# DankerMu/SHUD-up

Measured on AMD Instinct MI355X. Metric: element-flux-updates/sec (RHS evals × NumEle) at 1/2/4/8 GPUs; %HBM roofline, higher is better.
Workload: dtype f64

## Files before the change

shud-up_amd/csrc/shud_ele_packed.hip:

```cpp
#include <hip/hip_runtime.h>
#include <stdint.h>
#include <stdlib.h>

#include "shud_dev.h"
#include "shud_physics.h"

namespace shud {

typedef double v2d __attribute__((ext_vector_type(2)));
typedef int v4i __attribute__((ext_vector_type(4)));
template <class T>
__device__ __forceinline__ T ldnt(const T *p) { return __builtin_nontemporal_load(p); }
__device__ __forceinline__ double2 ldnt2(const double2 *p) {
    const v2d v = __builtin_nontemporal_load((const v2d *)p);
    return make_double2(v.x, v.y);
}
__device__ __forceinline__ int4 ldnt4(const int4 *p) {
    const v4i v = __builtin_nontemporal_load((const v4i *)p);
    return make_int4(v.x, v.y, v.z, v.w);
}
__device__ __forceinline__ void stnt2(double2 *p, double a, double b) {
    v2d v;
    v.x = a;
    v.y = b;
    __builtin_nontemporal_store(v, (v2d *)p);
}
template <class T>
__device__ __forceinline__ const T *at(const T *b, uint32_t off) { return (const T *)((const char *)b + off); }
template <class T>
__device__ __forceinline__ T *atw(T *b, uint32_t off) { return (T *)((char *)b + off); }

__device__ __forceinline__ bool nan_or_inf(double x) { return __builtin_isfpclass(x, 0x0003 | 0x0004 | 0x0200); }
__device__ __forceinline__ bool bad_nonneg(double x) {
    return __builtin_isfpclass(x, 0x0003 | 0x0004 | 0x0008 | 0x0010 | 0x0200);
}

__device__ __forceinline__ const double *riv_y_at(const YView &Y, int r) {
    return r < Y.n_own_riv ? Y.y + 3 * (size_t)Y.n_own + r : Y.griv + (r - Y.n_own_riv);
}

__device__ __forceinline__ int cf_ibc(int cf) { return (int)(int8_t)(cf & 0xff); }
__device__ __forceinline__ int cf_iss(int cf) { return (cf >> 8) & 3; }
__device__ __forceinline__ int cf_nseg(int cf) { return (cf >> 10) & 63; }
__device__ __forceinline__ int cf_class(int cf) { return (int)(((unsigned)cf >> 16) & 0x7fffu); }

template <int MODE>
__device__ __forceinline__ double ugw_pk(const DevMesh &m, double ygw_raw, int ibc, int j) {
    if (ibc == 0) return MODE == 0 ? ygw_raw : rmax(0.0, ygw_raw);
    if (ibc > 0) return m.eybc[ibc];
    return m.ugw_stale[j];
}

constexpr int LDS_CLS_MAX = kLdsClassMax;
constexpr int CF_LDS_STRIDE = CF_STRIDE;

constexpr int kEleWaves = 5;
constexpr int kEleWavesSh = 7;
constexpr bool kShareOn(bool lct, bool gh, bool lake, int hyb, bool diag) {
    return lct && !gh && !lake && hyb == 0 && !diag;
}
constexpr int kEleWavesOf(bool lct, int lspk, bool gh, bool lake, int hyb, bool diag, bool fu1, bool open) {
    return (kShareOn(lct, gh, lake, hyb, diag) && lspk) ? (fu1 ? kEleWavesSh : 6)
           : (kShareOn(lct, gh, lake, hyb, diag) && !open) ? 6 : kEleWaves;
}
constexpr int kEleBS = 256;
static_assert(kEleBS == kShareTile, "edge sharing pairs elements within one workgroup's tile");
static_assert(2 * kEleBS * 8 + kEleBS <= kPowTabDoubles * 8, "edge-sharing slots fit the pow tables' LDS region");
struct OwnRec {
    int4 mt;
    double2 zz, snp, stl, fu, csv;
    double ysf, yus, ygw;
    int sfl;
};
template <bool FU1, bool GH>
__device__ __forceinline__ OwnRec load_own(const DevPacked &p, const YView &Y, int i, int cur) {
    const int nown = Y.n_own;
    const uint32_t o16 = (uint32_t)i << 4, o8 = (uint32_t)i << 3;
    OwnRec o;
    o.mt = *at(p.meta, o16);
    o.zz = *at(p.zz, o16);
    o.ysf = GH ? Y.sf(i) : *at(Y.y, o8);
    o.yus = GH ? Y.us(i) : *at(Y.y + nown, o8);
    o.ygw = GH ? Y.gw(i) : *at(Y.y + 2 * (size_t)nown, o8);
    o.snp = ldnt2(at(p.s_np, o16));
    o.stl = ldnt2(at(p.s_tl, o16));
    if (FU1) { o.fu.x = 1.0; o.fu.y = 1.0; } else o.fu = ldnt2(at(p.s_fu, o16));
    o.csv = ldnt2(at(p.cs[cur], o16));
    o.sfl = *at(p.seg_first, (uint32_t)i << 2);
    return o;
}

constexpr int kTabBatch = 8;
template <int BS>
__device__ __forceinline__ void tab_issue(const DevPacked &p, double (&tv)[kTabBatch]) {
    const int nt2 = (p.ntab + 1) >> 1;
#pragma unroll
    for (int k = 0; k < kTabBatch / 2; k++) {
        const int t = (int)threadIdx.x + k * BS;
        const double2 v = t < nt2 ? ((const double2 *)p.ctab)[t] : make_double2(0., 0.);
        tv[2 * k] = v.x;
        tv[2 * k + 1] = v.y;
    }
}
template <int BS>
__device__ __forceinline__ void tab_store(const DevPacked &p, const double (&tv)[kTabBatch], double *lct) {
    const int nt2 = (p.ntab + 1) >> 1;
#pragma unroll
    for (int k = 0; k < kTabBatch / 2; k++) {
        const int t = (int)threadIdx.x + k * BS;
        if (t < nt2) ((double2 *)lct)[t] = make_double2(tv[2 * k], tv[2 * k + 1]);
    }
    for (int t = (int)threadIdx.x + kTabBatch / 2 * BS; t < nt2; t += BS)
        ((double2 *)lct)[t] = ((const double2 *)p.ctab)[t];
}
__device__ __forceinline__ int tile_of(int per8, int b) { return (b & 7) * per8 + (b >> 3); }
__device__ __forceinline__ int tile_of(int per8) { return tile_of(per8, (int)blockIdx.x); }
__device__ __forceinline__ bool share_idle_wave(bool act) {
    if (__builtin_amdgcn_ballot_w64(act)) return false;
    __syncthreads();
    __syncthreads();
    return true;
}

struct HaloWait;
template <int MODE, bool HALO>
__device__ __forceinline__ void qd_pre(const DevMesh &m, const DevPacked &p, const YView &Y, int r, int n_int,
                                       const HaloWait *hw);
__device__ __forceinline__ int qd_split(int b, int nb_q, int q0, int *e) {
    if (nb_q && b >= q0 && b < q0 + nb_q) return b - q0;
    *e = b < q0 ? b : b - nb_q;
    return -1;
}

template <int MODE, bool OPEN, bool DIAG, bool FU1, bool LCT, bool LAKE, bool GH, int HYB = 0, int LSP = 0, int BS = 256>
__device__ __forceinline__ void ele_body(const DevMesh &m, const DevPacked &p, const YView &Y, double *__restrict__ dy,
                                         int i, int cur, const DevDiag &dg, const DevLake &lk, const double *lct,
                                         const OwnRec &own);

template <int MODE, bool OPEN, bool DIAG, bool FU1, bool LCT, bool LAKE, bool GH, int HYB = 0, int LSPK = 0>
__global__ void __launch_bounds__(kEleBS, kEleWavesOf(LCT, LSPK, GH, LAKE, HYB, DIAG, FU1, OPEN))
shud_ele_kernel_packed(DevMesh m, DevPacked p, YView Y, double *__restrict__ dy, int i0, int n_compute, int cur,
                       DevDiag dg, DevLake lk, int per8, int nb_q, int q0) {
    extern __shared__ double lct[];
    int eb = (int)blockIdx.x;
    const int qb = qd_split((int)blockIdx.x, nb_q, q0, &eb);
    if (qb >= 0) {
        const int r = qb * kEleBS + (int)threadIdx.x;
        if (r < p.nqd) qd_pre<MODE, false>(m, p, Y, r, 0, nullptr);
        return;
    }
    const int i = i0 + tile_of(per8, eb) * kEleBS + (int)threadIdx.x;
    const bool act = i < n_compute;
    double tv[kTabBatch];
    if (LCT) tab_issue<kEleBS>(p, tv);
    OwnRec own;
    if (act) own = load_own<FU1, GH>(p, Y, i, cur);
    if (LCT) {
        tab_store<kEleBS>(p, tv, lct);
        __syncthreads();
    }
    if (kShareOn(LCT, GH, LAKE, HYB, DIAG) && LSPK != 0 && share_idle_wave(act)) return;
    if (act) ele_body<MODE, OPEN, DIAG, FU1, LCT, LAKE, GH, HYB, LCT ? LSPK : 0>(m, p, Y, dy, i, cur, dg, lk, lct, own);
}

template <int MODE, bool OPEN, bool DIAG, bool FU1, bool GH>
__global__ void __launch_bounds__(1024, 4)
shud_ele_kernel_packed_big(DevMesh m, DevPacked p, YView Y, double *__restrict__ dy, int i0, int n_compute, int cur,
                           DevDiag dg, DevLake lk, int per8) {
    extern __shared__ double lct[];
    const int i = i0 + tile_of(per8) * 1024 + (int)threadIdx.x;
    const bool act = i < n_compute;
    double tv[kTabBatch];
    tab_issue<1024>(p, tv);
    OwnRec own;
    if (act) own = load_own<FU1, GH>(p, Y, i, cur);
    tab_store<1024>(p, tv, lct);
    __syncthreads();
    if (act) ele_body<MODE, OPEN, DIAG, FU1, true, false, GH, 0, 0, 1024>(m, p, Y, dy, i, cur, dg, lk, lct, own);
}

__device__ __forceinline__ void halo_wait(const DevMesh &m, const HaloWait &hw, int i) {
    if (hw.epoch == 0) return;
    bool late = false;
    if (__lane_id() == 0) {
        const unsigned long long t0 = wall_clock64();
        while (__hip_atomic_load(hw.flag, __ATOMIC_RELAXED, __HIP_MEMORY_SCOPE_AGENT) < hw.epoch) {
            __builtin_amdgcn_s_sleep(8);
            if (wall_clock64() - t0 > hw.timeout) { late = true; break; }
        }
    }
    __builtin_amdgcn_fence(__ATOMIC_ACQUIRE, "agent");
    asm volatile("s_waitcnt vmcnt(0)" ::: "memory");
    report_w(m.err, late, 0x80u, 7, i);
}
template <int MODE, bool OPEN, bool FU1, int LSPK = 0>
__global__ void __launch_bounds__(256, (LSPK && FU1 && !OPEN) ? kEleWavesSh : kEleWaves)
shud_ele_kernel_packed_fold(DevMesh m, DevPacked p, YView Y, double *__restrict__ dy, int n_int, int n_all, int cur,
                            DevDiag dg, int per8, int nb_int, HaloWait hw, int nb_q, int q0) {
    extern __shared__ double lct[];
    const DevLake lk{};
    int b = (int)blockIdx.x;
    const int qb = qd_split((int)blockIdx.x, nb_q, q0, &b);
    if (qb >= 0) {
        const int r = qb * 256 + (int)threadIdx.x;
        qd_pre<MODE, true>(m, p, Y, r < p.nqd ? r : -1, n_int, &hw);
        return;
    }
    if (b < nb_int) {
        const int i = tile_of(per8, b) * 256 + (int)threadIdx.x;
        const bool act = i < n_int;
        double tv[kTabBatch];
        tab_issue<256>(p, tv);
        OwnRec own;
        if (act) own = load_own<FU1, false>(p, Y, i, cur);
        tab_store<256>(p, tv, lct);
        __syncthreads();
        if (LSPK != 0 && share_idle_wave(act)) return;
        if (act) ele_body<MODE, OPEN, false, FU1, true, false, false, 0, LSPK>(m, p, Y, dy, i, cur, dg, lk, lct, own);
        return;
    }
    const int i = n_int + (b - nb_int) * 256 + (int)threadIdx.x;
    const bool act = i < n_all;
    double tv[kTabBatch];
    tab_issue<256>(p, tv);
    halo_wait(m, hw, act ? i : n_int);
    OwnRec own;
    if (act) own = load_own<FU1, true>(p, Y, i, cur);
    tab_store<256>(p, tv, lct);
    __syncthreads();
    if (act) ele_body<MODE, OPEN, false, FU1, true, false, true, 0, LSPK ? 2 : 0>(m, p, Y, dy, i, cur, dg, lk, lct, own);
}
__global__ void shud_halo_flag_kernel(unsigned long long *flag, unsigned long long epoch) {
    if (threadIdx.x == 0) {
        __builtin_amdgcn_fence(__ATOMIC_RELEASE, "agent");
        asm volatile("s_waitcnt vmcnt(0)" ::: "memory");
        __hip_atomic_store(flag, epoch, __ATOMIC_RELAXED, __HIP_MEMORY_SCOPE_AGENT);
    }
}
__global__ void shud_spin_kernel(unsigned long long ticks) {
    if (threadIdx.x == 0) {
        const unsigned long long t0 = wall_clock64();
        while (wall_clock64() - t0 < ticks) __builtin_amdgcn_s_sleep(4);
    }
}
__global__ void shud_copy_f64_kernel(double *__restrict__ dst, const double *__restrict__ src, size_t n) {
    for (size_t k = blockIdx.x * (size_t)blockDim.x + threadIdx.x; k < n; k += (size_t)gridDim.x * blockDim.x)
        dst[k] = src[k];
}

__device__ __forceinline__ double hsel(const double (&v)[4], int k) {
    return k == 1 ? v[0] : k == 2 ? v[1] : k == 3 ? v[2] : v[3];
}
__device__ __forceinline__ void hload(const DevPacked &p, int i, double (&v)[4]) {
    v[1] = 0.; v[2] = 0.; v[3] = 0.;
    if (p.hs == 1) {
        v[0] = p.hv[i];
        return;
    }
    const double2 a = *(const double2 *)(p.hv + (size_t)p.hs * i);
    v[0] = a.x; v[1] = a.y;
    if (p.hs == 4) {
        const double2 b = *(const double2 *)(p.hv + (size_t)p.hs * i + 2);
        v[2] = b.x; v[3] = b.y;
    }
}

template <int MODE, bool OPEN, bool DIAG, bool FU1, bool LCT, bool LAKE, bool GH, int HYB, int LSP, int BS>
__device__ __forceinline__ void ele_body(const DevMesh &m, const DevPacked &p, const YView &Y, double *__restrict__ dy,
                                         int i, int cur, const DevDiag &dg, const DevLake &lk, const double *lct,
                                         const OwnRec &own) {
    const int NEl = m.num_ele;
    const int nown = Y.n_own;
    const uint32_t o16 = (uint32_t)i << 4, o8 = (uint32_t)i << 3;
    (void)o16;
    const int4 mt = own.mt;
    const double2 zz = own.zz;
    const double ysf_raw = own.ysf, yus_raw = own.yus, ygw_raw = own.ygw;
    const int cf = mt.w;
    const int cid = cf_class(cf), ibc = cf_ibc(cf);
    const bool is_lake = LAKE && cf < 0;
    const double2 snp = own.snp, stl = own.stl;
    const double etp = stl.y;
    const double2 fu = own.fu;
    const double2 csv = own.csv;
#define REPORT(c, bit, slot, cnt) report_w(m.err, (c), (bit), (slot), i, (cnt))
#define REPORT_ET(c, bit) (rep |= (c) ? (uint32_t)(bit) : 0u)
#define CL(f) (LCT ? lct[cid * CF_LDS_STRIDE + CfPos<CF_##f>::v] : p.ctab[cid * CF_STRIDE + CfPos<CF_##f>::v])
#define CDIV(a, F) cdiv(a, CL(F), CL(r_##F))
    double hvo[4] = {0., 0., 0., 0.};
    if (HYB == 1) hvo[0] = p.hv[i];
    else if (HYB == 2) hload(p, i, hvo);
#define CLH(f) ((HYB && p.hslot1[CF_##f]) ? (HYB == 1 ? hvo[0] : hsel(hvo, p.hslot1[CF_##f])) : CL(f))
#define CDIV_SY(a) ((HYB && p.hslot1[CF_Sy]) ? (a) / (HYB == 1 ? hvo[0] : hsel(hvo, p.hslot1[CF_Sy])) : CDIV(a, Sy))

    double usf = ysf_raw, uus = yus_raw;
    if (MODE == 1) { usf = (usf >= 0.) ? usf : 0.; uus = (uus >= 0.) ? uus : 0.; }
    const double ugw = ugw_pk<MODE>(m, ygw_raw, ibc, i);
    const double zs = zz.x, zb = zz.y;
    const double aq = zs - zb;

    double ekh, deficit, theta, satn, satkr;
    if (is_lake) {
        ekh = CLH(KsatH); deficit = 0.; satn = 1.; theta = CL(ThetaS); satkr = 1.0;
    } else {
        ekh = eff_kh(ugw, aq, CLH(macD), CLH(macKsatH), CLH(vAreaF), CLH(KsatH));
        REPORT(ekh < 0. || ekh > 1e9, 0x02u, 1, false);
        deficit = aq - ugw;
        const double ThS = CL(ThetaS), ThR = CL(ThetaR);
        if (deficit <= 0.) { deficit = 0.; satn = 1.; theta = ThS; }
        else { theta = uus / deficit * ThS; satn = CDIV(theta - ThR, dTh); }
        if (satn > 0.99) { satn = 1.0; satkr = 1.0; theta = ThS; }
        else if (satn <= K_ZERO) { satn = 0.; satkr = 0.; theta = ThR; }
        else {
            const double *pt = (LCT ? lct : p.ctab) + p.pt_off;
            satkr = sat_kfun(satn, CL(ex1), CL(ex2), pt, pt + kPowTabLogDoubles);
        }
    }

    const int sfl = own.sfl;
    const int sfirst = sfl & ((LSP || DIAG || !LCT) ? 0x03ffffff : 0x7fffffff);
    const bool lai_on = sfl < 0;
    const int iss = cf_iss(cf), nseg = cf_nseg(cf);
    const double infD = CL(infD), ThR = CL(ThetaR);
    const double infK = CL(infKsatV);
    const double fu_surf = fu.x, fu_sub = fu.y;

    double Es = 0., Eu = 0., Eg = 0., Tu = 0., Tg = 0., eic = csv.y, ibeta = 0.;
    if (is_lake) {
        eic = 0.;
        if (DIAG) { dg.q_es[i] = 0.; dg.q_eu[i] = 0.; dg.q_eg[i] = 0.; dg.q_tu[i] = 0.; dg.q_tg[i] = 0.;
                    dg.q_eta[i] = 0. + snp.y + 0.; }
    } else if (MODE == 0) {
        const double satn_prev = csv.x;
        const double va = CL(VegFrac), vb = 1. - va, pj = CL(pj);
        const double pet = snp.y, ptr = stl.x;
        ibeta = soil_moisture_stress(CDIV(satn_prev * CL(dTh) - ThR, fcmr));
        Es = rmin(rmax(0., usf), pet) * vb;
        if (Es < pet) {
            if (ugw > aq - infD) { Eg = rmin(rmax(0., ugw), pet - Es) * pj * vb; Eu = 0.; }
            else { Eg = 0.; Eu = rmin(rmax(0., uus), ibeta * (pet - Es)) * pj * vb; }
        }
        if (lai_on) {
            if (eic >= ptr) { Tg = Tu = 0.; eic = ptr * pj * va; }
            else if (ugw > aq - CLH(RzD)) { Tg = rmin(rmax(0., ugw), (ptr - eic)) * pj * va; Tu = 0.; }
            else { Tg = 0.; Tu = rmin(rmax(0., uus), ibeta * (ptr - eic)) * pj * va; }
        } else { Tg = Tu = eic = 0.; }
        const double trans = Tg + Tu, evapo = Eu + Eg + Es, eta = eic + evapo + trans;
        uint32_t rep = 0;
        REPORT_ET(eta > etp * 2., 0x10u);
        const bool neg = bad_nonneg(Es) || bad_nonneg(Eu) || bad_nonneg(Eg) || bad_nonneg(Tu) || bad_nonneg(Tg);
        REPORT_ET(neg, 0x04u);
        REPORT_ET(!neg && (nan_or_inf(eta) || nan_or_inf(evapo) || nan_or_inf(trans)), 0x08u);
        if (__builtin_amdgcn_ballot_w64(rep != 0)) {
            report_w(m.err, rep & 0x04u, 0x04u, 2, i);
            report_w(m.err, rep & 0x08u, 0x08u, 3, i);
            report_w(m.err, rep & 0x10u, 0x10u, 4, i, true);
        }
        if (DIAG) { dg.q_es[i] = Es; dg.q_eu[i] = Eu; dg.q_eg[i] = Eg; dg.q_tu[i] = Tu; dg.q_tg[i] = Tg;
                    dg.q_eta[i] = eta; dg.i_beta[i] = ibeta; }
    }
    stnt2(atw(p.cs[cur ^ 1], o16), satn, eic);

    double qi = 0., qex = 0., qr = 0.;
    if (!is_lake) {
        const double kmax = CL(kmax);
        const double av = usf + snp.x;
        if (ugw + uus > aq || deficit < uus) {
            qex = fabs(ugw + uus - aq) / aq * kmax;
        } else if (av > 0. && deficit > infD) {
            const double grad = 1. + CDIV(av, infD);
            double ek;
            if (av > kmax) ek = CL(ekA) + CL(ekB) * satn;
            else if (av > infK) ek = satkr * infK * CL(omh) + CL(ekB) * satn;
            else ek = satkr * infK * CL(omh);
            qi = rmin(av, rmax(0., grad * ek));
        }
        const double KV = CLH(KsatV);
        if (!(ugw > aq - infD && uus < deficit)) {
            double grad = 0.;
            if (theta > ThR && !(uus <= K_EPSILON)) {
                grad = CDIV(theta - ThR, fcmr);
                grad = rmax(grad, 0.);
            }
            if (!(infK <= 0. || KV <= 0.)) {
                const double ku = infK * satkr;
                qr = grad * ((ku * KV) * (deficit + ugw) / (deficit * KV + ugw * ku));
            }
        }
    }
    const double q_infil = qi * fu_surf, q_exfil = qex * fu_surf;
    const double q_rech = is_lake ? 0. : qr * fu_sub;

    const double dsf_head = snp.x - q_infil + q_exfil;
    const double dgw_head = q_rech - q_exfil;
    typedef __attribute__((address_space(3))) volatile double lds_vd;
    lds_vd *lsp = LSP ? (lds_vd *)(lct + p.ntab) + threadIdx.x : nullptr;
    typedef __attribute__((address_space(3))) volatile int lds_vi;
    lds_vi *lspi = LSP ? (lds_vi *)(lct + p.ntab + kLspN * kEleBS) + threadIdx.x : nullptr;
    if (LSP) {
        lsp[0] = Es; lsp[kEleBS] = Eg; lsp[2 * kEleBS] = Tg; lsp[3 * kEleBS] = dsf_head; lsp[4 * kEleBS] = dgw_head;
        lspi[0] = cf;
    }
    if (i < nown) __builtin_nontemporal_store(is_lake ? 0. : CDIV_SY(q_infil - q_rech - Eu - Tu), atw(dy + nown, o8));

    const double dep = CLH(depression), rgh = CLH(rough);
    double qe2r_surf = 0., qe2r_sub = 0.;
    if (nseg) {
        const double isf_seg = rmax(0., usf - q_infil + q_exfil);
        for (int k = sfirst, k1 = k + nseg; k < k1; k++) {
            const uint32_t k16 = (uint32_t)k << 4;
            const double2 lc = *at(p.sg_lc, k16);
            const int rr = *at(p.sg_r, (uint32_t)k << 2);
            const double2 dk = p.rrec[2 * (size_t)rr], rx = p.rrec[2 * (size_t)rr + 1];
            const int rbc = __builtin_bit_cast(int2, rx.y).x;
            const double bt = rx.x;
            double yr = GH ? Y.riv(rr) : *at(Y.y + 3 * (size_t)nown, (uint32_t)rr << 3);
            if (MODE == 1) yr = (yr >= 0.) ? yr : 0.;
            if (rbc > 0) yr = m.rybc[rbc];
            const double rdep = dk.x, L = lc.x;
            const double qs = weir_jtoi(zs, isf_seg, zs - rdep, yr, zs + 0.0, lc.y, L, dep);
            const double qg = r2e_gw(yr, zs - rdep, ugw, zb, ekh, dk.y, L, bt) * fu_sub;
            *atw(p.qseg2, k16) = make_double2(qs, qg);
            qe2r_surf += -qs;
            qe2r_sub += -qg;
        }
    }
    if (DIAG) {
        dg.q_infil[i] = q_infil; dg.q_exfil[i] = q_exfil; dg.q_recharge[i] = q_rech;
        dg.e_ic[i] = eic; dg.u_satn[i] = satn; dg.eff_kh[i] = ekh;
        dg.qe2r_surf[i] = qe2r_surf; dg.qe2r_sub[i] = qe2r_sub;
    }
    if (i >= nown) return;

    bool nan_q = false;
    const double isf = usf < 0. ? 0. : usf;
    const double area = ldnt(at(p.area, o8));
    const int n_edges = is_lake ? 0 : 3;
    constexpr bool SH = kShareOn(LCT, GH, LAKE, HYB, DIAG) && LSP != 0 && BS == kEleBS;
    constexpr bool DEC = !SH && LCT && !LAKE && HYB == 0 && BS == kEleBS && (LSP == 1 || DIAG);
    [[maybe_unused]] const uint32_t evo = (uint32_t)sfl >> kEvoShift;
    auto edge = [&](int s, int j, double &qsf, double &q, uint32_t &sh) __attribute__((always_inline)) {
        const int nb = s == 0 ? mt.x : s == 1 ? mt.y : mt.z;
        const int nc = nb >= 0 ? nb : i;
        const uint32_t n16 = (uint32_t)nc << 4, n8 = (uint32_t)nc << 3;
        const double2 g = ldnt2(at(p.ged, o16 + (uint32_t)s * ((uint32_t)NEl << 4)));
        const double2 nzz = *at(p.zz, n16);
        const int ncf = *at((const int *)p.meta + 3, n16);
        const double nsf_raw = GH ? Y.sf(nc) : *at(Y.y, n8);
        const double ngw_raw = GH ? Y.gw(nc) : *at(Y.y + 2 * (size_t)nown, n8);
        const double B = g.x, d2n = g.y;
        const Recip R2 = recip_nr(d2n);
        qsf = 0.; q = 0.; sh = 0u;
        const double dep_e = SH ? (double)((lds_vd *)lct)[cid * CF_LDS_STRIDE + CfPos<CF_depression>::v] : dep;
        const double rgh_e = SH ? (double)((lds_vd *)lct)[cid * CF_LDS_STRIDE + CfPos<CF_rough>::v] : rgh;
        const int cn = cf_class(ncf);
#define CN(f) (LCT ? lct[cn * CF_LDS_STRIDE + CfPos<CF_##f>::v] : p.ctab[cn * CF_STRIDE + CfPos<CF_##f>::v])
        double hvn[4] = {0., 0., 0., 0.};
        if (HYB == 1 && p.hnb) hvn[0] = p.hv[nc];
        else if (HYB == 2 && p.hnb) hload(p, nc, hvn);
#define CNH(f) ((HYB && p.hslot1[CF_##f]) ? (HYB == 1 ? hvn[0] : hsel(hvn, p.hslot1[CF_##f])) : CN(f))
        if (LAKE && nb >= 0 && ncf < 0) {
            const int l = lk.lake_of[nb];
            const double zl = lk.bathy_y[lk.bathy_off[l]];
            const double yl = Y.y[lk.y_off + l];
            const double nsf = yl < 0. ? 0. : yl;
            qsf = weir_jtoi(zl, nsf, zs, isf, zs, 0.6, B, 0.01);
            const double dhg = (ugw + zb) - (yl + zl);
            if (dhg > 0. && ugw <= 0.02) q = 0.;
            else if (dhg < 0. && yl <= 0.02) q = 0.;
            else {
                const double ymg = (rmax(ugw, 0.) + rmax(yl, 0.)) * .5;
                const double grad = div_nr(dhg, R2);
                const double kmean = 0.5 * (ekh + CNH(KsatH));
                q = kmean * grad * ymg * B;
            }
            lk.bank_qs[(size_t)j * NEl + i] = qsf;
            lk.bank_qg[(size_t)j * NEl + i] = q;
        } else if (nb >= 0) {
            double nsf = nsf_raw;
            if (MODE == 1) nsf = (nsf >= 0.) ? nsf : 0.;
            nsf = nsf < 0. ? 0. : nsf;
            const double zsn = nzz.x;
            const double dh = (isf + zs) - (nsf + zsn);
            [[maybe_unused]] const bool dh_nz = dh != 0., dh_ok = dh == dh;
            double ym = ((isf + zs) > (nsf + zsn)) ? ((isf > dep_e) ? isf : 0.) : ((nsf > dep_e) ? nsf : 0.);
            ym = rmin(ym, K_MAXYSURF);
            bool mu = false;
            if (ym > 0.) {
                const double s = div_nr(dh, R2);
                if (s > 0 && isf <= 0) qsf = 0.;
                else if (s < 0 && nsf <= 0) qsf = 0.;
                else { qsf = manning(ym * B, 0.5 * (rgh_e + CNH(rough)), ym, s); mu = true; }
            }
            const double ugn = ugw_pk<MODE>(m, ngw_raw, cf_ibc(ncf), nb);
            const double zbn = nzz.y;
            const double dhg = (ugw + zb) - (ugn + zbn);
            [[maybe_unused]] const bool dhg_nz = dhg != 0., dhg_ok = dhg == dhg;
            bool zq = true;
            if (dhg > 0. && ugw <= 0.02) q = 0.;
            else if (dhg < 0. && ugn <= 0.02) q = 0.;
            else {
                const double ekn = eff_kh(ugn, zsn - zbn, CNH(macD), CNH(macKsatH), CNH(vAreaF), CNH(KsatH));
                const double ymg = (rmax(ugw, 0.) + rmax(ugn, 0.)) * .5;
                const double grad = div_nr(dhg, R2);
                const double kmean = 0.5 * (ekh + ekn);
                q = kmean * grad * ymg * B;
                zq = false;
            }
            if constexpr (SH) sh = (mu && dh_nz ? 1u : 0u) | (!zq && dhg_nz ? 2u : 0u) | (dh_ok && dhg_ok ? 4u : 0u);
        } else if (OPEN) {
            const double d2e = m.dist2edge[(SH ? evo_ref(evo, s) : j) * NEl + i];
            if (isf > dep_e) {
                const double s = isf / d2e * 0.5;
                if (s > 0.) qsf = sqrt(s) * cbrt(isf * isf * isf * isf * isf) * B / rgh_e;
            }
            if (ugw > dep_e * 10.) {
                const double grad = ugw / d2e * 0.5;
                if (grad > 0.) q = ekh * grad;
            }
        }
#undef CN
#undef CNH
    };
    double sumsurf = qe2r_surf, sumsub = qe2r_sub;
    auto add = [&](int j, double qsf, double q) __attribute__((always_inline)) {
        const double qsb = q * fu_sub;
        if (MODE == 0) nan_q |= nan_or_inf(qsf) || nan_or_inf(qsb);
        sumsurf += qsf;
        sumsub += qsb;
        if (DIAG) { dg.qele_surf[j * NEl + i] = qsf; dg.qele_sub[j * NEl + i] = qsb; }
    };
    if constexpr (!SH) {
#pragma unroll 1
        for (int j = 0; j < n_edges; j++) {
            double qsf, q;
            uint32_t sh;
            edge(DEC ? evo_stored(evo, j) : j, j, qsf, q, sh);
            add(j, qsf, q);
        }
    } else {
        typedef __attribute__((address_space(3))) volatile unsigned char lds_vb;
        lds_vd *xq = (lds_vd *)(lct + p.pt_off);
        lds_vb *xf = (lds_vb *)(lct + p.pt_off + 2 * kEleBS);
        const int tid = (int)threadIdx.x;
        __syncthreads();
        {
            double qsf, q;
            uint32_t sh;
            edge(0, 0, qsf, q, sh);
            xq[tid] = qsf;
            xq[kEleBS + tid] = q;
            xf[tid] = (unsigned char)sh;
        }
        __syncthreads();
        double a1, b1, a2 = 0., b2 = 0.;
        {
            uint32_t sh;
            edge(1, 1, a1, b1, sh);
        }
        bool own2 = true;
        if (evo & (kEvoRcv2 >> kEvoShift)) {
            const int rt = mt.z - (i - tid);
            if (rt >= 0 && rt < kEleBS) {
                const uint32_t f = xf[rt];
                if (f & 4u) {
                    const double a = xq[rt], b = xq[kEleBS + rt];
                    a2 = (f & 1u) ? -a : a;
                    b2 = (f & 2u) ? -b : b;
                    own2 = false;
                }
            }
        }
        if (__builtin_amdgcn_ballot_w64(own2)) {
            if (own2) {
                uint32_t sh;
                edge(2, 2, a2, b2, sh);
            }
        }
        const double a0 = xq[tid], b0 = xq[kEleBS + tid];
        const uint32_t s0 = evo & 3u;
        const bool sw = (evo & 4u) != 0;
        const double la = s0 == 0 ? a1 : a0, lb = s0 == 0 ? b1 : b0;
        const double ha = s0 == 2 ? a1 : a2, hb = s0 == 2 ? b1 : b2;
        add(0, s0 == 0 ? a0 : s0 == 1 ? a1 : a2, s0 == 0 ? b0 : s0 == 1 ? b1 : b2);
        add(1, sw ? ha : la, sw ? hb : lb);
        add(2, sw ? la : ha, sw ? lb : hb);
    }
    if (DIAG && is_lake)
        for (int j = 0; j < 3; j++) { dg.qele_surf[j * NEl + i] = 0.; dg.qele_sub[j * NEl + i] = 0.; }
    if (MODE == 0) REPORT(nan_q, 0x01u, 0, false);

    double dsf, dgw;
    const Recip RA = recip_nr(area);
    if (LSP) {
        const double es = lsp[0], eg = lsp[kEleBS], tg = lsp[2 * kEleBS], dsh = lsp[3 * kEleBS], dgh = lsp[4 * kEleBS];
        dsf = dsh - div_nr(sumsurf, RA) - es;
        dgw = dgh - div_nr(sumsub, RA) - eg - tg;
    } else {
        dsf = dsf_head - div_nr(sumsurf, RA) - Es;
        dgw = dgw_head - div_nr(sumsub, RA) - Eg - Tg;
    }
    const int cf_t = LSP ? lspi[0] : cf;
    const int ibc_t = LSP ? cf_ibc(cf_t) : ibc, iss_t = LSP ? cf_iss(cf_t) : iss;
    if (ibc_t > 0) dgw = 0;
    else if (ibc_t < 0) dgw += div_nr(m.eqbc[-ibc_t], RA);
    if (iss_t == 1) dsf += zero_over(area);
    else if (iss_t == 2) dgw += zero_over(area);
    dgw = CDIV_SY(dgw);
    if (LSP ? (LAKE && cf_t < 0) : is_lake) { dsf = 0.; dgw = 0.; }
#undef CL
#undef CLH
#undef CDIV_SY
    __builtin_nontemporal_store(dsf, atw(dy, o8));
    __builtin_nontemporal_store(dgw, atw(dy + 2 * (size_t)nown, o8));
    if (DIAG) { dg.qele_surf_tot[i] = sumsurf; dg.qele_sub_tot[i] = sumsub; }
#undef REPORT
#undef REPORT_ET
}

struct RivP {
    double w0, bs, len, slope, d2d, n, depth;
    int down, bc;
};
__device__ __forceinline__ int2 rv_ib(double x) { return __builtin_bit_cast(int2, x); }
__device__ __forceinline__ RivP riv_load(const DevPacked &p, int r) {
    const double2 *q = p.rv + 4 * (size_t)r;
    const double2 a = q[0], b = q[1], c = q[2], d = q[3];
    const int2 ib = rv_ib(d.y);
    RivP o;
    o.w0 = a.x; o.bs = a.y; o.len = b.x; o.slope = b.y; o.d2d = c.x; o.n = c.y; o.depth = d.x;
    o.down = ib.x; o.bc = ib.y;
    return o;
}
__device__ __forceinline__ RivGeom riv_geom_p(const RivP &q, double y) { return riv_geom(q.w0, q.bs, q.len, y); }
template <int MODE>
__device__ __forceinline__ double riv_stage_p(const DevMesh &m, const YView &Y, int r, int bc, double *yg) {
    double yr = Y.riv(r);
    if (MODE == 1) yr = (yr >= 0.) ? yr : 0.;
    *yg = yr;
    return bc > 0 ? m.rybc[bc] : yr;
}
__device__ __forceinline__ double riv_down_p(const RivP &q, double uq, const RivGeom &g, double ud, double ddepth,
                                             double dslope) {
    if (q.down >= 0) {
        const double smean = (q.slope + dslope) * 0.5;
        const double s = ((uq - q.depth) - (ud - ddepth)) / q.d2d + smean;
        const double R = (g.csperem <= K_ZERO) ? 0. : (g.csarea / g.csperem);
        return manning(g.csarea, q.n, R, s);
    } else if (q.down >= -3) {
        const double s = q.slope + uq * 2. / q.len;
        const double R = (g.csperem <= 0.) ? 0. : (g.csarea / g.csperem);
        return manning(g.csarea, q.n, R, s);
    }
    return g.csarea * sqrt(K_GRAV * uq) * 60.;
}
__device__ __forceinline__ double riv_down_outlet(const RivP &q, double uq, const RivGeom &g) {
    return riv_down_p(q, uq, g, 0., 0., 0.);
}
template <int MODE, bool HALO>
__device__ __forceinline__ void qd_pre(const DevMesh &m, const DevPacked &p, const YView &Y, int r, int n_int,
                                       const HaloWait *hw) {
    const int rr = r < 0 ? 0 : r;
    const RivP q = riv_load(p, rr);
    const int d = q.down >= 0 ? q.down : rr;
    if (HALO) {
        const bool ghost = r >= 0 && (r >= Y.n_own_riv || d >= Y.n_own_riv);
        if (__builtin_amdgcn_ballot_w64(ghost)) halo_wait(m, *hw, n_int);
    }
    if (r < 0) return;
    double yg;
    const double ur = riv_stage_p<MODE>(m, Y, r, q.bc, &yg);
    const RivGeom g = riv_geom_p(q, yg);
    const double2 bd = p.rv[4 * (size_t)d + 1], dd = p.rv[4 * (size_t)d + 3];
    double ydg;
    const double ud = riv_stage_p<MODE>(m, Y, d, rv_ib(dd.y).y, &ydg);
    p.qdown[r] = riv_down_p(q, ur, g, ud, dd.x, bd.y);
}

struct __attribute__((packed, aligned(4))) Int4u { int x, y, z, w; };
struct __attribute__((packed, aligned(4))) Int2u { int x, y; };

template <int MODE, bool DIAG, int SB, bool QD>
__device__ __forceinline__ void riv_body(const DevMesh &m, const DevPacked &p, const YView &Y, double *__restrict__ dy,
                                         const DevDiag &dg, int r) {
    const RivP q = riv_load(p, r);
    const int4 ru = p.rv_u[r];
    const int seg0 = ru.x, nseg = ru.y & 0xffff, upc = ru.y >> 16;
    double yg;
    const double ur = riv_stage_p<MODE>(m, Y, r, q.bc, &yg);
    const RivGeom g = riv_geom_p(q, yg);
    double qdown = 0.;
    if (QD) {
        qdown = p.qdown[r];
    } else {
        const int d = q.down >= 0 ? q.down : r;
        const double2 bd = p.rv[4 * (size_t)d + 1], dd = p.rv[4 * (size_t)d + 3];
        const int bcd = rv_ib(dd.y).y;
        double ydg;
        const double ud = riv_stage_p<MODE>(m, Y, d, bcd, &ydg);
        qdown = riv_down_p(q, ur, g, ud, dd.x, bd.y);
    }
    auto up_term = [&](int u) {
        if (QD) return -p.qdown[u];
        const RivP qu = riv_load(p, u);
        double yu;
        const double uu = riv_stage_p<MODE>(m, Y, u, qu.bc, &yu);
        return -riv_down_p(qu, uu, riv_geom_p(qu, yu), ur, q.depth, q.slope);
    };
    double qup = 0.;
    if (upc < 3) {
        if (upc > 0) qup += up_term(ru.z);
        if (upc > 1) qup += up_term(ru.w);
    } else {
        for (int k0 = ru.z, k1 = ru.z + ru.w; k0 < k1; k0 += 8) {
            int uv[8];
#pragma unroll
            for (int j = 0; j < 8; j++) uv[j] = m.up_idx[k0 + j < k1 ? k0 + j : k0];
#pragma unroll
            for (int j = 0; j < 8; j++)
                if (k0 + j < k1) qup += up_term(uv[j]);
        }
    }
    double qsurf = 0., qsub = 0.;
    for (int k0 = seg0, k1 = seg0 + nseg; k0 < k1; k0 += SB) {
        int raw[SB], ps[SB];
#pragma unroll
        for (int c = 0; c + 4 <= SB; c += 4) {
            const Int4u v = *reinterpret_cast<const Int4u *>(m.rseg_pos + k0 + c);
            raw[c] = v.x; raw[c + 1] = v.y; raw[c + 2] = v.z; raw[c + 3] = v.w;
        }
        if constexpr (SB % 4 == 2) {
            const Int2u v = *reinterpret_cast<const Int2u *>(m.rseg_pos + k0 + SB - 2);
            raw[SB - 2] = v.x; raw[SB - 1] = v.y;
        }
#pragma unroll
        for (int j = 0; j < SB; j++) ps[j] = k0 + j < k1 ? raw[j] : raw[0];
        double2 qv[SB];
#pragma unroll
        for (int j = 0; j < SB; j++) qv[j] = p.qseg2[ps[j]];
#pragma unroll
        for (int j = 0; j < SB; j++)
            if (k0 + j < k1) { qsurf += qv[j].x; qsub += qv[j].y; }
    }
    const double qbc = (q.bc < 0) ? m.rqbc[-q.bc] : 0.0;
    double dv;
    if (q.bc > 0) dv = 0.;
    else if (MODE == 0) {
        dv = (-qup - qsurf - qsub - qdown + qbc) / q.len;
        if (dv < -1. * g.csarea) dv = -1. * g.csarea;
        dv = da_to_dy(dv, g.topw, q.bs);
    } else {
        dv = (-qup - qsurf - qsub - qdown + qbc) / g.toparea;
    }
    dy[3 * Y.n_own + r] = dv;
    if (DIAG) { dg.qriv_down[r] = qdown; dg.qriv_up[r] = qup; dg.qriv_surf[r] = qsurf; dg.qriv_sub[r] = qsub; }
}
template <int MODE, bool DIAG, int SB, bool QD>
__global__ void __launch_bounds__(256)
shud_riv_kernel_packed(DevMesh m, DevPacked p, YView Y, double *__restrict__ dy, DevDiag dg, int per8) {
    const int r = tile_of(per8) * 256 + (int)threadIdx.x;
    if (r >= Y.n_own_riv) return;
    riv_body<MODE, DIAG, SB, QD>(m, p, Y, dy, dg, r);
}

template <int SB, bool QD>
static void launch_riv_sb(const DevMesh &m, const DevPacked &p, const YView &Y, double *dy, int mode, bool diag,
                          const DevDiag &dg, hipStream_t s) {
    const dim3 grid(((Y.n_own_riv + 255) / 256 + 7) / 8 * 8), blk(256);
    const int per8 = (int)grid.x / 8;
    if (mode == 0) {
        if (diag) hipLaunchKernelGGL((shud_riv_kernel_packed<0, true, SB, QD>), grid, blk, 0, s, m, p, Y, dy, dg, per8);
        else hipLaunchKernelGGL((shud_riv_kernel_packed<0, false, SB, QD>), grid, blk, 0, s, m, p, Y, dy, dg, per8);
    } else {
        if (diag) hipLaunchKernelGGL((shud_riv_kernel_packed<1, true, SB, QD>), grid, blk, 0, s, m, p, Y, dy, dg, per8);
        else hipLaunchKernelGGL((shud_riv_kernel_packed<1, false, SB, QD>), grid, blk, 0, s, m, p, Y, dy, dg, per8);
    }
}

void launch_river_kernel_packed(const DevMesh &m, const DevPacked &p, const YView &Y, double *dy, int mode,
                                bool diag, const DevDiag &dg, hipStream_t s, bool qd) {
    if (Y.n_own_riv <= 0) return;
    const int sb = p.riv_sb;
    if (qd && p.qdown) {
        if (sb == 6) launch_riv_sb<6, true>(m, p, Y, dy, mode, diag, dg, s);
        else launch_riv_sb<8, true>(m, p, Y, dy, mode, diag, dg, s);
    } else {
        if (sb == 6) launch_riv_sb<6, false>(m, p, Y, dy, mode, diag, dg, s);
        else launch_riv_sb<8, false>(m, p, Y, dy, mode, diag, dg, s);
    }
}

__device__ double lake_toparea(const DevLake &L, int l, double y) {
    const double *yi = L.bathy_y + L.bathy_off[l], *ai = L.bathy_a + L.bathy_off[l];
    const int nvalue = L.bathy_off[l + 1] - L.bathy_off[l];
    double ta = ai[0];
    if (y <= yi[0]) {
        ta = ai[0];
    } else {
        for (int k = 1; k < nvalue; k++) {
            if (y < yi[k]) {
                const double da = (ai[k] - ta), dyy = yi[k] - y;
                ta = da / dyy * (y - yi[k - 1]) + ta;
                break;
            }
            ta = ai[k];
        }
    }
    return ta;
}

template <class F>
__device__ double ordered_sum(int k0, int k1, F f, double *buf) {
    double acc = 0.;
    for (int b = k0; b < k1; b += blockDim.x) {
        const int k = b + (int)threadIdx.x;
        if (k < k1) buf[threadIdx.x] = f(k);
        __syncthreads();
        if (threadIdx.x == 0) {
            const int n = min((int)blockDim.x, k1 - b);
            for (int t = 0; t < n; t++) acc += buf[t];
        }
        __syncthreads();
    }
    return acc;
}

__global__ void __launch_bounds__(256)
shud_lake_kernel(DevMesh m, DevPacked p, DevLake L, YView Y, double *__restrict__ dy, int diag, DevDiag dg) {
    __shared__ double buf[256];
    const int l = blockIdx.x;
    const double yl = Y.y[L.y_off + l];
    const int e0 = L.ele_off[l], e1 = L.ele_off[l + 1];
    const double n_ele = (double)(e1 - e0);
    const double qevap = ordered_sum(e0, e1, [&](int k) { return m.pot_evap[L.ele_idx[k]] / n_ele; }, buf);
    const double qprcp = ordered_sum(e0, e1, [&](int k) { return m.prcp[L.ele_idx[k]] / n_ele; }, buf);
    const double qsurf = ordered_sum(L.bank_off[l], L.bank_off[l + 1],
                                     [&](int k) { return L.bank_qs[L.bank_pos[k]]; }, buf);
    const double qsub = ordered_sum(L.bank_off[l], L.bank_off[l + 1],
                                    [&](int k) { return L.bank_qg[L.bank_pos[k]]; }, buf);
    const double qin = ordered_sum(L.rin_off[l], L.rin_off[l + 1], [&](int k) {
        const int r = L.rin_idx[k];
        const RivP q = riv_load(p, r);
        double yg;
        const double ur = riv_stage_p<0>(m, Y, r, q.bc, &yg);
        return riv_down_outlet(q, ur, riv_geom_p(q, yg));
    }, buf);
    if (threadIdx.x == 0) {
        const double zmin = L.bathy_y[L.bathy_off[l]];
        const double area = lake_toparea(L, l, yl + zmin);
        double qe = rmin(qevap, qprcp + yl);
        qe = rmax(0, qe);
        dy[L.y_off + l] = qprcp - qe + (qin - 0. + qsub + qsurf) / area;
        if (diag) {
            dg.q_lake_surf[l] = qsurf; dg.q_lake_sub[l] = qsub; dg.q_lake_rivin[l] = qin;
            dg.q_lake_evap[l] = qe; dg.q_lake_prcp[l] = qprcp; dg.lake_toparea[l] = area;
        }
    }
}

void launch_lake_kernel(const DevMesh &m, const DevPacked &p, const DevLake &L, const YView &Y, double *dy,
                        bool diag, const DevDiag &dg, hipStream_t s) {
    if (L.nl <= 0) return;
    hipLaunchKernelGGL(shud_lake_kernel, dim3(L.nl), dim3(256), 0, s, m, p, L, Y, dy, diag ? 1 : 0, dg);
}

__global__ void __launch_bounds__(256)
shud_pack_step_kernel(DevMesh m, DevPacked p, int n, int cur, unsigned what) {
    const int i = blockIdx.x * blockDim.x + threadIdx.x;
    if (i >= n) return;
    if (what & 1) p.s_np[i] = make_double2(m.net_prep[i], m.pot_evap[i]);
    if (what & 2) {
        p.s_tl[i] = make_double2(m.pot_tran[i], m.etp[i]);
        p.seg_first[i] = (p.seg_first[i] & 0x7fffffff) | (m.lai[i] > K_ZERO ? (int)0x80000000u : 0);
    }
    if (what & 4) p.s_fu[i] = make_double2(m.fu_surf[i], m.fu_sub[i]);
    if (what & 8) p.cs[cur][i].x = m.u_satn[0][i];
    if (what & 16) p.cs[cur][i].y = m.e_ic[0][i];
}

template <int MODE, bool OPEN, bool DIAG, bool FU1, bool GH>
static void launch_big(const DevMesh &m, const DevPacked &p, const YView &Y, double *dy, int i0, int i1, int cur,
                       const DevDiag &dg, const DevLake &lk, hipStream_t s) {
    int nb = (i1 - i0 + 1023) / 1024;
    nb = (nb + 7) / 8 * 8;
    const size_t lds = (size_t)p.ntab * sizeof(double);
    auto *fn = shud_ele_kernel_packed_big<MODE, OPEN, DIAG, FU1, GH>;
    static bool attr = false;
    if (!attr) {
        (void)hipFuncSetAttribute((const void *)fn, hipFuncAttributeMaxDynamicSharedMemorySize,
                                  (int)((kLdsClassMaxBig * CF_LDS_STRIDE + 1 + kPowTabDoubles) * sizeof(double)));
        attr = true;
    }
    hipLaunchKernelGGL(fn, dim3(nb), dim3(1024), lds, s, m, p, Y, dy, i0, i1, cur, dg, lk, nb / 8);
}

static int qd_start(int nb, int pm) {
    const long long q = (long long)nb * std::min(std::max(pm, 0), 1000) / 1000;
    return (int)(q / 8 * 8);
}
static size_t lds_bytes(const DevPacked &p, bool lct, bool lspk) {
    if (!lct) return 0;
    return lspk ? lsp_lds_bytes(p.ntab) : (size_t)p.ntab * sizeof(double);
}
template <int MODE, bool OPEN, bool DIAG, bool FU1, bool LCT, bool LAKE, bool GH, int HYB = 0, int LSPK = 0>
static void launch_p(const DevMesh &m, const DevPacked &p, const YView &Y, double *dy, int i0, int i1, int cur,
                     const DevDiag &dg, const DevLake &lk, hipStream_t s, int nq = 0) {
    int nb = (i1 - i0 + kEleBS - 1) / kEleBS;
    nb = (nb + 7) / 8 * 8;
    const int nbq = nq > 0 ? ((nq + kEleBS - 1) / kEleBS + 7) / 8 * 8 : 0;
    const int q0 = qd_start(nb, p.qd_pm);
    const size_t lds = lds_bytes(p, LCT, LSPK != 0);
    hipLaunchKernelGGL((shud_ele_kernel_packed<MODE, OPEN, DIAG, FU1, LCT, LAKE, GH, HYB, LSPK>), dim3(nb + nbq), dim3(kEleBS),
                       lds, s,
                       m, p, Y, dy, i0, i1, cur, dg, lk, nb / 8, nbq, q0);
}

template <int MO, bool OP, bool DI, bool FU, bool GH>
static void launch_plain(const DevMesh &m, const DevPacked &p, const YView &Y, double *dy, int i0, int i1, int cur,
                         const DevDiag &dg, const DevLake &lk, hipStream_t s, int nq) {
    if constexpr (!DI) {
        if (lds_bytes(p, true, true) <= kLspLdsMax) {
            launch_p<MO, OP, DI, FU, true, false, GH, 0, 1>(m, p, Y, dy, i0, i1, cur, dg, lk, s, nq);
            return;
        }
    }
    launch_p<MO, OP, DI, FU, true, false, GH>(m, p, Y, dy, i0, i1, cur, dg, lk, s, nq);
}
bool launch_element_kernel_packed(const DevMesh &m, const DevPacked &p, const YView &Y, double *dy, int i0, int i1,
                                  int cur, int mode, bool open, bool diag, bool fu_unit, const DevDiag &dg,
                                  hipStream_t s, const DevLake *lake, bool interior, bool with_qd) {
    if (i1 <= i0) return false;
    DevLake lk{};
    if (lake) lk = *lake;
    const int nq = (with_qd && p.qdown && p.nqd > 0 && (lake || p.ncls <= LDS_CLS_MAX)) ? p.nqd : 0;
    const bool gh = !interior && (Y.gele != nullptr || Y.griv != nullptr);
#define LP(MO, OP, DI, FU) do {                                                                            \
        if (lake && MO == 0) {                                                                            \
            if (gh) launch_p<MO, OP, DI, FU, true, true, true>(m, p, Y, dy, i0, i1, cur, dg, lk, s, nq);  \
            else launch_p<MO, OP, DI, FU, true, true, false>(m, p, Y, dy, i0, i1, cur, dg, lk, s, nq);    \
        }                                                                                                 \
        else if (p.ncls > LDS_CLS_MAX && p.ncls <= kLdsClassMaxBig && p.lds_big) {                        \
            if (gh) launch_big<MO, OP, DI, FU, true>(m, p, Y, dy, i0, i1, cur, dg, lk, s);                 \
            else launch_big<MO, OP, DI, FU, false>(m, p, Y, dy, i0, i1, cur, dg, lk, s);                   \
        }                                                                                                 \
        else if (p.ncls <= LDS_CLS_MAX && p.nh == 1) {                                                    \
            if (gh) launch_p<MO, OP, DI, FU, true, false, true, 1>(m, p, Y, dy, i0, i1, cur, dg, lk, s, nq); \
            else launch_p<MO, OP, DI, FU, true, false, false, 1>(m, p, Y, dy, i0, i1, cur, dg, lk, s, nq);   \
        }                                                                                                 \
        else if (p.ncls <= LDS_CLS_MAX && p.nh) {                                                         \
            if (gh) launch_p<MO, OP, DI, FU, true, false, true, 2>(m, p, Y, dy, i0, i1, cur, dg, lk, s, nq); \
            else launch_p<MO, OP, DI, FU, true, false, false, 2>(m, p, Y, dy, i0, i1, cur, dg, lk, s, nq);   \
        }                                                                                                 \
        else if (p.ncls <= LDS_CLS_MAX) {                                                                 \
            if (gh) launch_plain<MO, OP, DI, FU, true>(m, p, Y, dy, i0, i1, cur, dg, lk, s, nq);          \
            else launch_plain<MO, OP, DI, FU, false>(m, p, Y, dy, i0, i1, cur, dg, lk, s, nq);            \
        } else launch_p<MO, OP, DI, FU, false, false, true>(m, p, Y, dy, i0, i1, cur, dg, lk, s); } while (0)
#define LFU(MO, OP, DI) do { if (fu_unit) LP(MO, OP, DI, true); else LP(MO, OP, DI, false); } while (0)
#define LDI(MO, OP) do { if (diag) LFU(MO, OP, true); else LFU(MO, OP, false); } while (0)
#define LOP(MO) do { if (open) LDI(MO, true); else LDI(MO, false); } while (0)
    if (mode == 0) LOP(0); else LOP(1);
#undef LOP
#undef LDI
#undef LFU
#undef LP
    return nq > 0;
}

bool launch_element_kernel_packed_fold(const DevMesh &m, const DevPacked &p, const YView &Y, double *dy, int n_int,
                                       int n_all, int cur, int mode, bool open, bool fu_unit, const DevDiag &dg,
                                       const HaloWait &hw, hipStream_t s, bool with_qd) {
    if (n_int <= 0 || n_all <= n_int || p.ncls > LDS_CLS_MAX || p.nh) return false;
    const int nb_int = ((n_int + 255) / 256 + 7) / 8 * 8, nb_b = (n_all - n_int + 255) / 256;
    const int nbq = (with_qd && p.qdown && p.nqd > 0) ? ((p.nqd + 255) / 256 + 7) / 8 * 8 : 0;
    const int q0 = qd_start(nb_int, p.qd_pm_fold);
    const bool lsp = lds_bytes(p, true, true) <= kLspLdsMax;
    const size_t lds = lds_bytes(p, true, lsp);
#define LF(MO, OP, FU) do {                                                                                        \
        if (lsp) hipLaunchKernelGGL((shud_ele_kernel_packed_fold<MO, OP, FU, 1>),                \
                                    dim3(nb_int + nb_b + nbq), dim3(256), lds, s, m, p, Y, dy, n_int, n_all, cur, dg, \
                                    nb_int / 8, nb_int, hw, nbq, q0);                                              \
        else hipLaunchKernelGGL((shud_ele_kernel_packed_fold<MO, OP, FU>), dim3(nb_int + nb_b + nbq), dim3(256),    \
                                lds, s, m, p, Y, dy, n_int, n_all, cur, dg, nb_int / 8, nb_int, hw, nbq, q0);       \
    } while (0)
    if (mode == 0) {
        if (open) { if (fu_unit) LF(0, true, true); else LF(0, true, false); }
        else { if (fu_unit) LF(0, false, true); else LF(0, false, false); }
    } else {
        if (open) { if (fu_unit) LF(1, true, true); else LF(1, true, false); }
        else { if (fu_unit) LF(1, false, true); else LF(1, false, false); }
    }
#undef LF
    return true;
}
void launch_halo_flag(unsigned long long *flag, unsigned long long epoch, hipStream_t s) {
    hipLaunchKernelGGL(shud_halo_flag_kernel, dim3(1), dim3(64), 0, s, flag, epoch);
}
void launch_spin(unsigned long long ticks, hipStream_t s) {
    hipLaunchKernelGGL(shud_spin_kernel, dim3(1), dim3(64), 0, s, ticks);
}
void launch_copy_f64(double *dst, const double *src, size_t n, hipStream_t s) {
    if (!n) return;
    const size_t nb = std::min<size_t>((n + 255) / 256, 4096);
    hipLaunchKernelGGL(shud_copy_f64_kernel, dim3((unsigned)nb), dim3(256), 0, s, dst, src, n);
}

void launch_pack_step_kernel(const DevMesh &m, const DevPacked &p, int n, int cur, unsigned what, hipStream_t s) {
    if (n <= 0 || !what) return;
    hipLaunchKernelGGL(shud_pack_step_kernel, dim3((n + 255) / 256), dim3(256), 0, s, m, p, n, cur, what);
}

}
```

Measured before the change: 19.61 billion.

## Prefetch first river segment and edge neighbor loads ahead of barriers

Splits the segment and edge computations into a load phase and an evaluate phase. In the edge-sharing path, the first river segment's record and river state are fetched before the infiltration math, and the edge 0/1 neighbor loads and the area load are issued before the workgroup barriers. The goal is to hide global memory latency behind computation and synchronisation. In exchange, more values stay live across the barriers, and empty asm constraints are used to pin them in VGPRs, which raises register pressure and may reduce occupancy.

```diff
diff --git a/shud-up_amd/csrc/shud_ele_packed.hip b/shud-up_amd/csrc/shud_ele_packed.hip
--- a/shud-up_amd/csrc/shud_ele_packed.hip
+++ b/shud-up_amd/csrc/shud_ele_packed.hip
@@ -66,6 +66,17 @@
 constexpr int kEleBS = 256;
 static_assert(kEleBS == kShareTile, "edge sharing pairs elements within one workgroup's tile");
 static_assert(2 * kEleBS * 8 + kEleBS <= kPowTabDoubles * 8, "edge-sharing slots fit the pow tables' LDS region");
+struct SegIn {
+    int rr;
+    double2 lc, dk, rx;
+    double yr;
+};
+struct EdgeIn {
+    int nb;
+    double2 g, nzz;
+    int ncf;
+    double nsf_raw, ngw_raw;
+};
 struct OwnRec {
     int4 mt;
     double2 zz, snp, stl, fu, csv;
@@ -321,6 +332,18 @@
     const int sfirst = sfl & ((LSP || DIAG || !LCT) ? 0x03ffffff : 0x7fffffff);
     const bool lai_on = sfl < 0;
     const int iss = cf_iss(cf), nseg = cf_nseg(cf);
+    auto seg_a = [&](int k, SegIn &si) __attribute__((always_inline)) {
+        si.rr = *at(p.sg_r, (uint32_t)k << 2);
+        si.lc = *at(p.sg_lc, (uint32_t)k << 4);
+    };
+    auto seg_b = [&](SegIn &si) __attribute__((always_inline)) {
+        const int rr = si.rr;
+        si.dk = p.rrec[2 * (size_t)rr];
+        si.rx = p.rrec[2 * (size_t)rr + 1];
+        si.yr = GH ? Y.riv(rr) : *at(Y.y + 3 * (size_t)nown, (uint32_t)rr << 3);
+    };
+    constexpr bool SEG_EARLY = kShareOn(LCT, GH, LAKE, HYB, DIAG) && LSP != 0 && BS == kEleBS;
+    SegIn sg0 = {};
     const double infD = CL(infD), ThR = CL(ThetaR);
     const double infK = CL(infKsatV);
     const double fu_surf = fu.x, fu_sub = fu.y;
@@ -360,6 +383,7 @@
                     dg.q_eta[i] = eta; dg.i_beta[i] = ibeta; }
     }
     stnt2(atw(p.cs[cur ^ 1], o16), satn, eic);
+    if (SEG_EARLY && nseg) seg_a(sfirst, sg0);
 
     double qi = 0., qex = 0., qr = 0.;
     if (!is_lake) {
@@ -401,28 +425,37 @@
         lsp[0] = Es; lsp[kEleBS] = Eg; lsp[2 * kEleBS] = Tg; lsp[3 * kEleBS] = dsf_head; lsp[4 * kEleBS] = dgw_head;
         lspi[0] = cf;
     }
+    if (SEG_EARLY && nseg) seg_b(sg0);
     if (i < nown) __builtin_nontemporal_store(is_lake ? 0. : CDIV_SY(q_infil - q_rech - Eu - Tu), atw(dy + nown, o8));
 
     const double dep = CLH(depression), rgh = CLH(rough);
     double qe2r_surf = 0., qe2r_sub = 0.;
+    if (SEG_EARLY)
+        asm volatile("" ::"v"(sg0.lc.x), "v"(sg0.lc.y), "v"(sg0.dk.x), "v"(sg0.dk.y), "v"(sg0.rx.x),
+                     "v"(__builtin_bit_cast(int2, sg0.rx.y).x), "v"(sg0.yr));
     if (nseg) {
         const double isf_seg = rmax(0., usf - q_infil + q_exfil);
-        for (int k = sfirst, k1 = k + nseg; k < k1; k++) {
-            const uint32_t k16 = (uint32_t)k << 4;
-            const double2 lc = *at(p.sg_lc, k16);
-            const int rr = *at(p.sg_r, (uint32_t)k << 2);
-            const double2 dk = p.rrec[2 * (size_t)rr], rx = p.rrec[2 * (size_t)rr + 1];
-            const int rbc = __builtin_bit_cast(int2, rx.y).x;
-            const double bt = rx.x;
-            double yr = GH ? Y.riv(rr) : *at(Y.y + 3 * (size_t)nown, (uint32_t)rr << 3);
+        auto seg_flux = [&](int k, const SegIn &si) __attribute__((always_inline)) {
+            const int rbc = __builtin_bit_cast(int2, si.rx.y).x;
+            const double bt = si.rx.x;
+            double yr = si.yr;
+            asm volatile("" : "+v"(yr));
             if (MODE == 1) yr = (yr >= 0.) ? yr : 0.;
             if (rbc > 0) yr = m.rybc[rbc];
-            const double rdep = dk.x, L = lc.x;
-            const double qs = weir_jtoi(zs, isf_seg, zs - rdep, yr, zs + 0.0, lc.y, L, dep);
-            const double qg = r2e_gw(yr, zs - rdep, ugw, zb, ekh, dk.y, L, bt) * fu_sub;
-            *atw(p.qseg2, k16) = make_double2(qs, qg);
+            const double rdep = si.dk.x, L = si.lc.x;
+            const double qs = weir_jtoi(zs, isf_seg, zs - rdep, yr, zs + 0.0, si.lc.y, L, dep);
+            const double qg = r2e_gw(yr, zs - rdep, ugw, zb, ekh, si.dk.y, L, bt) * fu_sub;
+            *atw(p.qseg2, (uint32_t)k << 4) = make_double2(qs, qg);
             qe2r_surf += -qs;
             qe2r_sub += -qg;
+        };
+        if (SEG_EARLY) seg_flux(sfirst, sg0);
+#pragma unroll 1
+        for (int k = sfirst + (SEG_EARLY ? 1 : 0), k1 = sfirst + nseg; k < k1; k++) {
+            SegIn si;
+            seg_a(k, si);
+            seg_b(si);
+            seg_flux(k, si);
         }
     }
     if (DIAG) {
@@ -434,20 +467,31 @@
 
     bool nan_q = false;
     const double isf = usf < 0. ? 0. : usf;
-    const double area = ldnt(at(p.area, o8));
     const int n_edges = is_lake ? 0 : 3;
     constexpr bool SH = kShareOn(LCT, GH, LAKE, HYB, DIAG) && LSP != 0 && BS == kEleBS;
+    double area = 0.;
+    if (!SH) area = ldnt(at(p.area, o8));
     constexpr bool DEC = !SH && LCT && !LAKE && HYB == 0 && BS == kEleBS && (LSP == 1 || DIAG);
     [[maybe_unused]] const uint32_t evo = (uint32_t)sfl >> kEvoShift;
-    auto edge = [&](int s, int j, double &qsf, double &q, uint32_t &sh) __attribute__((always_inline)) {
-        const int nb = s == 0 ? mt.x : s == 1 ? mt.y : mt.z;
-        const int nc = nb >= 0 ? nb : i;
+    auto edge_load = [&](int s) __attribute__((always_inline)) {
+        EdgeIn e;
+        e.nb = s == 0 ? mt.x : s == 1 ? mt.y : mt.z;
+        const int nc = e.nb >= 0 ? e.nb : i;
         const uint32_t n16 = (uint32_t)nc << 4, n8 = (uint32_t)nc << 3;
-        const double2 g = ldnt2(at(p.ged, o16 + (uint32_t)s * ((uint32_t)NEl << 4)));
-        const double2 nzz = *at(p.zz, n16);
-        const int ncf = *at((const int *)p.meta + 3, n16);
-        const double nsf_raw = GH ? Y.sf(nc) : *at(Y.y, n8);
-        const double ngw_raw = GH ? Y.gw(nc) : *at(Y.y + 2 * (size_t)nown, n8);
+        e.g = ldnt2(at(p.ged, o16 + (uint32_t)s * ((uint32_t)NEl << 4)));
+        e.nzz = *at(p.zz, n16);
+        e.ncf = *at((const int *)p.meta + 3, n16);
+        e.nsf_raw = GH ? Y.sf(nc) : *at(Y.y, n8);
+        e.ngw_raw = GH ? Y.gw(nc) : *at(Y.y + 2 * (size_t)nown, n8);
+        return e;
+    };
+    auto edge_eval = [&](int s, int j, const EdgeIn &e, double &qsf, double &q, uint32_t &sh)
+                         __attribute__((always_inline)) {
+        const int nb = e.nb;
+        [[maybe_unused]] const int nc = nb >= 0 ? nb : i;
+        const double2 g = e.g, nzz = e.nzz;
+        const int ncf = e.ncf;
+        const double nsf_raw = e.nsf_raw, ngw_raw = e.ngw_raw;
         const double B = g.x, d2n = g.y;
         const Recip R2 = recip_nr(d2n);
         qsf = 0.; q = 0.; sh = 0u;
@@ -522,6 +566,10 @@
 #undef CN
 #undef CNH
     };
+    auto edge = [&](int s, int j, double &qsf, double &q, uint32_t &sh) __attribute__((always_inline)) {
+        const EdgeIn e = edge_load(s);
+        edge_eval(s, j, e, qsf, q, sh);
+    };
     double sumsurf = qe2r_surf, sumsub = qe2r_sub;
     auto add = [&](int j, double qsf, double q) __attribute__((always_inline)) {
         const double qsb = q * fu_sub;
@@ -543,20 +591,23 @@
         lds_vd *xq = (lds_vd *)(lct + p.pt_off);
         lds_vb *xf = (lds_vb *)(lct + p.pt_off + 2 * kEleBS);
         const int tid = (int)threadIdx.x;
+        const EdgeIn e0 = edge_load(0);
+        area = ldnt(at(p.area, o8));
         __syncthreads();
         {
             double qsf, q;
             uint32_t sh;
-            edge(0, 0, qsf, q, sh);
+            edge_eval(0, 0, e0, qsf, q, sh);
             xq[tid] = qsf;
             xq[kEleBS + tid] = q;
             xf[tid] = (unsigned char)sh;
         }
+        const EdgeIn e1 = edge_load(1);
         __syncthreads();
         double a1, b1, a2 = 0., b2 = 0.;
         {
             uint32_t sh;
-            edge(1, 1, a1, b1, sh);
+            edge_eval(1, 1, e1, a1, b1, sh);
         }
         bool own2 = true;
         if (evo & (kEvoRcv2 >> kEvoShift)) {
```

After: 19.99 billion (median of 6 runs). +1.9%, better.
